# zouyuoz/SVS-UNet-PyTorch

Measured on AMD Instinct MI355X. Metric: spectrogram-tiles/sec (512x128) U-Net fwd+bwd (L1 train step incl. Adam), higher is better.
Workload: dtype f32; 1 GPU; train.py L1-loss step, 512x128 tiles, batch 64 per GPU; global_batch=64, parallelism=dp1, mode=train

## Files before the change

### svs_unet_pytorch_amd/csrc/gemm_conv.hip

```cpp
#include <stdlib.h>
#include <string.h>

#include <mutex>
#include <type_traits>
#include <vector>
#include "common.h"
#include "mfma_split.h"

enum { MODE_GATHER = 0, MODE_PARITY = 1 };

struct ConvGemmArgs {
  const float* x; long ldx;
  int B, H, W, C;
  const float* wp;
  const float* bias;
  const float* scale;
  const float* shift;
  float slope;
  float* y; long ldy;
  int Ho, Wo, N;
  int accumulate;
  int ksplit;
  float* slab;
  int tap_inner;
  int cpt_shift;
  float* stats;
};

struct ConvBal {
  int enabled;
  int npos[4];
  unsigned first[4][65];
  unsigned char nsplit[4][64];
  unsigned char* rowsplit;
};
struct ConvNoBal {};

__device__ __forceinline__ int swz(int row, int chunk) { return chunk ^ ((row >> 1) & 3); }

template <int MODE, int BM, int BN, int WM, int WN, bool SKIP = false, bool SPLIT = false, int PF = 1>
__global__ __launch_bounds__(256) void conv_gemm_kernel(ConvGemmArgs p, std::conditional_t<SKIP, ConvBal, ConvNoBal> bal) {
  constexpr int TM = BM / WM / 16;
  constexpr int TN = BN / WN / 16;
  constexpr int RA = (BM + 63) / 64;
  constexpr int RB = (BN + 63) / 64;
  static_assert(WM * WN == 4, "4 waves");
  static_assert(TM >= 1 && TN >= 1, "tile");

  __shared__ __attribute__((aligned(16))) float As[2][BM * 16];
  __shared__ __attribute__((aligned(16))) float Bs[2][BN * 16];

  const int t = threadIdx.x;
  const int lane = t & 63, wave = t >> 6;
  const int wm = wave / WN, wn = wave % WN;
  const int lrow = lane & 15, q = lane >> 4;

  int bx = blockIdx.x, by = blockIdx.y, bz = blockIdx.z;
  int nsplit = p.ksplit;
  bool balanced = false;
  if constexpr (SKIP) {
    if (bal.enabled) {
      balanced = true;
      const unsigned bid = blockIdx.x;
      int c = 0;
      if (MODE == MODE_PARITY) c = (bid >= bal.first[1][0]) + (bid >= bal.first[2][0]) + (bid >= bal.first[3][0]);
      const unsigned f = lane < bal.npos[c] ? bal.first[c][lane] : 0xFFFFFFFFu;
      const int pos = __builtin_amdgcn_readfirstlane(__builtin_popcountll(__ballot(f <= bid)) - 1);
      nsplit = bal.nsplit[c][pos];
      const int ntn = p.N / BN, per = nsplit * ntn;
      const int within = (int)(bid - bal.first[c][pos]);
      const int i = within / per, rem = within - i * per;
      by = rem / ntn;
      bx = (pos * (p.B / BM) + i) * ntn + (rem - by * ntn);
      bz = c;
    }
  }
  int ph = 0, pw = 0, nth = 5, ntw = 5;
  int Ha, Wa;
  const float* wp = p.wp;
  if (MODE == MODE_PARITY) {
    const int par = bz;
    ph = par >> 1; pw = par & 1;
    nth = 3 - ph; ntw = 3 - pw;
    Ha = (p.Ho - ph + 1) >> 1; Wa = (p.Wo - pw + 1) >> 1;
    const int poff = (par == 0) ? 0 : (par == 1) ? 9 : (par == 2) ? 15 : 21;
    wp += (long)poff * p.N * p.C;
  } else {
    Ha = p.Ho; Wa = p.Wo;
  }
  const int ntaps = nth * ntw;
  const long M = (long)p.B * Ha * Wa;
  const int ntile_n = p.N / BN;
  const long m0 = (long)(bx / ntile_n) * BM;
  const int n0 = (bx % ntile_n) * BN;
  if (m0 >= M) {
    if (p.stats && p.ksplit == 1) {
      float* out = p.stats + ((long)bz * (gridDim.x / ntile_n) + bx / ntile_n) * 2 * p.N + n0;
      for (int c = threadIdx.x; c < BN; c += 256) { out[c] = 0.f; out[p.N + c] = 0.f; }
    }
    return;
  }
  const int cpt = p.C >> 4;
  const int nkt = ntaps * cpt;
  int kt_begin = (int)((long)nkt * by / nsplit);
  int kt_end = (int)((long)nkt * (by + 1) / nsplit);
  const long Kw = (long)ntaps * p.C;

  const int chunk = t & 3;
  constexpr unsigned OOB = 0x80000000u;
  unsigned a_voff[RA], a_mask[RA];
#pragma unroll
  for (int r = 0; r < RA; ++r) {
    const int row = (t >> 2) + 64 * r;
    const long m = m0 + row;
    const bool ok = (row < BM) && (m < M);
    const long mm = ok ? m : 0;
    int wq, hq; long b;
    if (SKIP) {
      const unsigned pos = (unsigned)mm / (unsigned)p.B;
      b = (long)((unsigned)mm - pos * (unsigned)p.B);
      wq = (int)(pos / (unsigned)Ha);
      hq = (int)(pos - (unsigned)wq * (unsigned)Ha);
    } else {
      const unsigned um = (unsigned)mm, utmp = um / (unsigned)Wa;
      wq = (int)(um - utmp * (unsigned)Wa);
      const unsigned ub = utmp / (unsigned)Ha;
      hq = (int)(utmp - ub * (unsigned)Ha);
      b = ub;
    }
    const int h0 = (MODE == MODE_GATHER) ? 2 * hq : hq;
    const int w0 = (MODE == MODE_GATHER) ? 2 * wq : wq;
    a_voff[r] = ok ? (unsigned)((((b * p.H + h0) * p.W + w0) * p.ldx + chunk * 4) * 4) : OOB;
    unsigned mask = 0;
    for (int th = 0; th < nth; ++th)
      for (int tw = 0; tw < ntw; ++tw) {
        const int ih = (MODE == MODE_GATHER) ? h0 - 2 + th : h0 + 1 - th;
        const int iw = (MODE == MODE_GATHER) ? w0 - 2 + tw : w0 + 1 - tw;
        if (ok && (unsigned)ih < (unsigned)p.H && (unsigned)iw < (unsigned)p.W) mask |= 1u << (th * ntw + tw);
      }
    a_mask[r] = mask;
  }
  unsigned umask = 0x1FFFFFFu;
  if (SKIP) {
    __shared__ unsigned umask_s;
    if (t == 0) umask_s = 0;
    __syncthreads();
    unsigned mine = 0;
#pragma unroll
    for (int r = 0; r < RA; ++r) mine |= a_mask[r];
    if (mine) atomicOr(&umask_s, mine);
    __syncthreads();
    umask = __builtin_amdgcn_readfirstlane(umask_s);
    if (balanced) {
      const int nvk = __builtin_popcount(umask) << p.cpt_shift;
      const int vb = (int)((long)nvk * by / nsplit), ve = (int)((long)nvk * (by + 1) / nsplit);
      auto kt_of = [&](int v) -> int {
        unsigned m = umask;
        for (int r = v >> p.cpt_shift; r > 0; --r) m &= m - 1;
        return (__builtin_ctz(m) << p.cpt_shift) | (v & (cpt - 1));
      };
      kt_begin = vb < nvk ? kt_of(vb) : nkt;
      kt_end = ve < nvk ? kt_of(ve) : nkt;
    }
  }
  unsigned b_voff[RB];
#pragma unroll
  for (int r = 0; r < RB; ++r) {
    const int row = (t >> 2) + 64 * r;
    b_voff[r] = (row < BN) ? (unsigned)(((long)(n0 + row) * Kw + chunk * 4) * 4) : OOB;
  }
  const long shift = (MODE == MODE_GATHER) ? (2L * p.W + 2) * p.ldx : (1L * p.W + 1) * p.ldx;
  const __amdgpu_buffer_rsrc_t rx = __builtin_amdgcn_make_buffer_rsrc((void*)(p.x - shift), 0, OOB, 0x00020000);
  const __amdgpu_buffer_rsrc_t rw = __builtin_amdgcn_make_buffer_rsrc((void*)wp, 0, OOB, 0x00020000);

  f32x4 ra[RA], rb[RB];
  f32x4 ra2[PF == 2 ? RA : 1], rb2[PF == 2 ? RB : 1];
  auto load_tile_to = [&](int kt, f32x4 (&ra)[RA], f32x4 (&rb)[RB]) __attribute__((always_inline)) {
    int tap, cc;
    if (SKIP || !p.tap_inner) {
      if (p.cpt_shift >= 0) { tap = kt >> p.cpt_shift; cc = kt & (cpt - 1); }
      else { tap = kt / cpt; cc = kt - tap * cpt; }
    } else {
      cc = (ntaps == 25) ? kt / 25 : (ntaps == 9) ? kt / 9 : (ntaps == 6) ? kt / 6 : kt >> 2;
      tap = kt - cc * ntaps;
    }
    const int th = (ntw == 5) ? tap / 5 : (ntw == 3) ? tap / 3 : tap >> 1;
    const int tw = tap - th * ntw;
    const int pix = (MODE == MODE_GATHER) ? th * p.W + tw : (2 - th) * p.W + (2 - tw);
    const int soff_a = __builtin_amdgcn_readfirstlane((int)((pix * p.ldx + (cc << 4)) * 4));
    const int soff_b = __builtin_amdgcn_readfirstlane((int)(((long)tap * p.C + (cc << 4)) * 4));
#pragma unroll
    for (int r = 0; r < RA; ++r) {
      const unsigned vo = ((a_mask[r] >> tap) & 1u) ? a_voff[r] : OOB;
      ra[r] = __builtin_bit_cast(f32x4, __builtin_amdgcn_raw_buffer_load_b128(rx, (int)vo, soff_a, 0));
    }
#pragma unroll
    for (int r = 0; r < RB; ++r)
      rb[r] = __builtin_bit_cast(f32x4, __builtin_amdgcn_raw_buffer_load_b128(rw, (int)b_voff[r], soff_b, 0));
  };
  auto load_tile = [&](int kt) __attribute__((always_inline)) { load_tile_to(kt, ra, rb); };
  auto store_tile_from = [&](int buf, const f32x4 (&ra)[RA], const f32x4 (&rb)[RB]) __attribute__((always_inline)) {
#pragma unroll
    for (int r = 0; r < RA; ++r) {
      const int row = (t >> 2) + 64 * r;
      if (BM % 64 == 0 || row < BM) *(f32x4*)(&As[buf][row * 16 + swz(row, chunk) * 4]) = ra[r];
    }
#pragma unroll
    for (int r = 0; r < RB; ++r) {
      const int row = (t >> 2) + 64 * r;
      if (BN % 64 == 0 || row < BN) *(f32x4*)(&Bs[buf][row * 16 + swz(row, chunk) * 4]) = rb[r];
    }
  };

  auto store_tile = [&](int buf) __attribute__((always_inline)) { store_tile_from(buf, ra, rb); };
  f32x4 acc[TM][TN];
#pragma unroll
  for (int i = 0; i < TM; ++i)
#pragma unroll
    for (int j = 0; j < TN; ++j) acc[i][j] = (f32x4){0.f, 0.f, 0.f, 0.f};

  auto first_valid = [&](int k) -> int {
    if (!SKIP || k >= kt_end) return k;
    const int tp = k >> p.cpt_shift;
    if ((umask >> tp) & 1u) return k;
    const unsigned rest = umask >> (tp + 1);
    if (!rest) return kt_end;
    const int nk = (tp + 1 + __builtin_ctz(rest)) << p.cpt_shift;
    return nk < kt_end ? nk : kt_end;
  };
  auto multiply = [&](int buf) __attribute__((always_inline)) {
    f32x4 fa[TM], fb[TN];
#pragma unroll
    for (int i = 0; i < TM; ++i) {
      const int row = wm * (TM * 16) + i * 16 + lrow;
      fa[i] = *(const f32x4*)(&As[buf][row * 16 + swz(row, q) * 4]);
    }
#pragma unroll
    for (int j = 0; j < TN; ++j) {
      const int row = wn * (TN * 16) + j * 16 + lrow;
      fb[j] = *(const f32x4*)(&Bs[buf][row * 16 + swz(row, q) * 4]);
    }
    if constexpr (SPLIT) {
      SvsSplitA sa[TM];
      SvsSplitB sb[TN];
#pragma unroll
      for (int i = 0; i < TM; ++i) sa[i] = svs_split_a(fa[i][0], fa[i][1], fa[i][2], fa[i][3]);
// ... 34 lines not shown
    }
  } else {
  if (kt_cur < kt_end) {
    load_tile(kt_cur);
    store_tile(0);
  }
  __syncthreads();
  for (int it = 0; kt_cur < kt_end; ++it) {
    const int buf = it & 1;
    const int kt_next = first_valid(kt_cur + 1);
    const bool more = kt_next < kt_end;
    if (more) load_tile(kt_next);
    kt_cur = kt_next;
    f32x4 fa[TM], fb[TN];
#pragma unroll
    for (int i = 0; i < TM; ++i) {
      const int row = wm * (TM * 16) + i * 16 + lrow;
      fa[i] = *(const f32x4*)(&As[buf][row * 16 + swz(row, q) * 4]);
    }
#pragma unroll
    for (int j = 0; j < TN; ++j) {
      const int row = wn * (TN * 16) + j * 16 + lrow;
      fb[j] = *(const f32x4*)(&Bs[buf][row * 16 + swz(row, q) * 4]);
    }
    if constexpr (SPLIT) {
      SvsSplitA sa[TM];
      SvsSplitB sb[TN];
#pragma unroll
      for (int i = 0; i < TM; ++i) sa[i] = svs_split_a(fa[i][0], fa[i][1], fa[i][2], fa[i][3]);
#pragma unroll
      for (int j = 0; j < TN; ++j) sb[j] = svs_split_b(fb[j][0], fb[j][1], fb[j][2], fb[j][3]);
      svs_mma_split<TM, TN>(acc, sa, sb);
    } else {
#pragma unroll
      for (int k = 0; k < 4; ++k)
#pragma unroll
        for (int i = 0; i < TM; ++i)
#pragma unroll
          for (int j = 0; j < TN; ++j)
            acc[i][j] = __builtin_amdgcn_mfma_f32_16x16x4f32(fa[i][k], fb[j][k], acc[i][j], 0, 0, 0);
    }
    if (more) store_tile(buf ^ 1);
    __syncthreads();
  }
  }

  const bool split = p.ksplit > 1;
  float ssum[TN], ssq[TN];
#pragma unroll
  for (int j = 0; j < TN; ++j) { ssum[j] = 0.f; ssq[j] = 0.f; }
  float* const slab = split ? p.slab + (long)by * ((long)p.B * p.Ho * p.Wo) * p.N : nullptr;
  bool mark_rows = false;
  if constexpr (SKIP) mark_rows = balanced && by == 0 && n0 == 0 && wn == 0;
#pragma unroll
  for (int i = 0; i < TM; ++i) {
#pragma unroll
    for (int r = 0; r < 4; ++r) {
      const long m = m0 + wm * (TM * 16) + i * 16 + q * 4 + r;
      if (m >= M) continue;
      long opix;
      if (SKIP) {
        const unsigned pos = (unsigned)m / (unsigned)p.B;
        const long b = (long)((unsigned)m - pos * (unsigned)p.B);
        const int wq = (int)(pos / (unsigned)Ha);
        const int hq = (int)(pos - (unsigned)wq * (unsigned)Ha);
        opix = (MODE == MODE_GATHER) ? (b * p.Ho + hq) * p.Wo + wq : (b * p.Ho + 2 * hq + ph) * p.Wo + 2 * wq + pw;
      } else if (MODE == MODE_GATHER) {
        opix = m;
      } else {
        const unsigned um = (unsigned)m, utmp = um / (unsigned)Wa;
        const int wq = (int)(um - utmp * (unsigned)Wa);
        const unsigned ub = utmp / (unsigned)Ha;
        const int hq = (int)(utmp - ub * (unsigned)Ha);
        const long b = ub;
        opix = (b * p.Ho + 2 * hq + ph) * p.Wo + 2 * wq + pw;
      }
      if constexpr (SKIP) { if (mark_rows && lrow == 0) bal.rowsplit[opix] = (unsigned char)nsplit; }
#pragma unroll
      for (int j = 0; j < TN; ++j) {
        const int n = n0 + wn * (TN * 16) + j * 16 + lrow;
        float v = acc[i][j][r];
        if (split) {
          slab[opix * p.N + n] = v;
        } else {
          if (p.bias) v += p.bias[n];
          if (p.scale) {
            v = v * p.scale[n] + p.shift[n];
            v = v > 0.f ? v : v * p.slope;
          }
          float* dst = p.y + opix * p.ldy + n;
          if (p.accumulate) v += *dst;
          *dst = v;
          ssum[j] += v;
          ssq[j] += v * v;
        }
      }
    }
  }
  if (p.stats && !split) {
    __shared__ float st[2][WM][BN];
#pragma unroll
    for (int j = 0; j < TN; ++j) {
      ssum[j] += __shfl_xor(ssum[j], 16, 64); ssum[j] += __shfl_xor(ssum[j], 32, 64);
      ssq[j] += __shfl_xor(ssq[j], 16, 64); ssq[j] += __shfl_xor(ssq[j], 32, 64);
      if (q == 0) { st[0][wm][wn * (TN * 16) + j * 16 + lrow] = ssum[j]; st[1][wm][wn * (TN * 16) + j * 16 + lrow] = ssq[j]; }
    }
    __syncthreads();
    float* out = p.stats + ((long)bz * (gridDim.x / ntile_n) + bx / ntile_n) * 2 * p.N + n0;
    for (int c = t; c < BN; c += 256) {
      float a = 0.f, b2 = 0.f;
#pragma unroll
      for (int w = 0; w < WM; ++w) { a += st[0][w][c]; b2 += st[1][w][c]; }
      out[c] = a;
      out[p.N + c] = b2;
    }
  }
}

template <int MODE, int TM, int TN>
__global__ __launch_bounds__(256) void conv_direct_kernel(ConvGemmArgs p) {
  const int t = threadIdx.x;
  const int lane = t & 63, wave = t >> 6;
  const int lrow = lane & 15, q = lane >> 4;
  int ph = 0, pw = 0, nth = 5, ntw = 5, Ha, Wa;
  const float* wp = p.wp;
  if (MODE == MODE_PARITY) {
    const int par = blockIdx.y;
    ph = par >> 1; pw = par & 1;
    nth = 3 - ph; ntw = 3 - pw;
    Ha = (p.Ho - ph + 1) >> 1; Wa = (p.Wo - pw + 1) >> 1;
    const int poff = (par == 0) ? 0 : (par == 1) ? 9 : (par == 2) ? 15 : 21;
    wp += (long)poff * p.N * p.C;
  } else {
    Ha = p.Ho; Wa = p.Wo;
  }
  const int ntaps = nth * ntw;
  const long M = (long)p.B * Ha * Wa;
  const long m0 = ((long)blockIdx.x * 4 + wave) * (TM * 16);
  if (m0 >= M) return;
  const int cpt = p.C >> 4;
  const int nkt = ntaps * cpt;
  const long Kw = (long)ntaps * p.C;
  constexpr unsigned OOB = 0x80000000u;

  unsigned a_voff[TM], a_mask[TM];
#pragma unroll
  for (int i = 0; i < TM; ++i) {
    const long m = m0 + i * 16 + lrow;
    const bool ok = m < M;
    const long mm = ok ? m : 0;
// ... 456 lines not shown
#pragma unroll
    for (int i = 0; i < 4; ++i) acc[i] = (f32x4){0.f, 0.f, 0.f, 0.f};
    f32x4 fw[2];
    fw[0] = __builtin_bit_cast(f32x4, __builtin_amdgcn_raw_buffer_load_b128(rw, (int)w_voff, 0, 0));
    svs_static_for<25>([&](auto tc) {
      constexpr int tap = decltype(tc)::value, kh = tap / 5, kw = tap % 5;
      if constexpr (tap + 1 < 25) fw[(tap + 1) & 1] = __builtin_bit_cast(f32x4, __builtin_amdgcn_raw_buffer_load_b128(rw, (int)w_voff, (tap + 1) * 16 * 4, 0));
      f32x4 fp[4];
#pragma unroll
      for (int i = 0; i < 4; ++i) fp[i] = *(const f32x4*)(pbase + (((2 * i + kh) * 2 + (kw & 1)) * PW + (kw >> 1)) * LP);
#pragma unroll
      for (int k = 0; k < 4; ++k)
#pragma unroll
        for (int i = 0; i < 4; ++i) acc[i] = __builtin_amdgcn_mfma_f32_16x16x4f32(fw[tap & 1][k], fp[i][k], acc[i], 0, 0, 0);
    });
#pragma unroll
    for (int i = 0; i < 4; ++i) {
      const int oh = oh0 + 4 * rh + i, ow = ow0 + lrow;
      if (oh >= p.Ho || ow >= p.Wo) continue;
      f32x4 v = acc[i];
      if (p.bias) v += b4;
      if (p.scale) {
        v = v * sc4 + sh4;
#pragma unroll
        for (int k = 0; k < 4; ++k) v[k] = v[k] > 0.f ? v[k] : v[k] * p.slope;
      }
      *(f32x4*)(p.y + ((b * p.Ho + oh) * p.Wo + ow) * p.ldy + n) = v;
      s0 += v;
      s1 += v * v;
    }
  }
  if (p.stats) {
#pragma unroll
    for (int k = 0; k < 4; ++k)
#pragma unroll
      for (int o = 1; o < 16; o <<= 1) { s0[k] += __shfl_xor(s0[k], o, 64); s1[k] += __shfl_xor(s1[k], o, 64); }
    if (lrow == 0) {
#pragma unroll
      for (int k = 0; k < 4; ++k) { st[0][rh][n + k] = s0[k]; st[1][rh][n + k] = s1[k]; }
    }
    __syncthreads();
    if (t < 64) {
      const int which = t >> 5, c = t & 31;
      p.stats[(long)blockIdx.x * 64 + which * 32 + c] = st[which][0][c] + st[which][1][c];
    }
  }
}

enum ConvKind { CONV_GEMM, CONV_GATHER_WINDOW, CONV_PARITY_WINDOW, CONV_DIRECT };
struct ConvPlan {
  int kind;
  int cfg, BM, BN, WM, WN, pf;
  bool skip, split;
  long mtiles; int grid_y;
  int wC, wCW, wTN, wNT;
  bool wvec;
  int tpb, gtiles;
  dim3 grid;
  int ksplit;
  ConvBal bal;
  size_t slab_bytes, rowtab_bytes;
  long stat_rows;
};

static void plan_gemm_tile(int mode, long Mmax, int N, int nkt_min, bool narrow, bool inference, ConvPlan& pl) {
  if (N % 128 == 0) {
    if (Mmax <= 96) { pl.cfg = 4; pl.BM = 32; pl.BN = 128; }
    else { pl.cfg = 0; pl.BM = 128; pl.BN = 128; }
  } else if (N == 64) {
    if (Mmax <= 512 || nkt_min <= 25 || (inference && Mmax <= 16384)) { pl.cfg = 5; pl.BM = 64; pl.BN = 64; }
    else { pl.cfg = 1; pl.BM = 128; pl.BN = 64; }
  } else if (N == 32) { pl.cfg = 2; pl.BM = 256; pl.BN = 32; }
  else { pl.cfg = 3; pl.BM = 256; pl.BN = 16; }
  if (mode == MODE_PARITY && N % 64 == 0 && Mmax > 1024) { pl.cfg = 5; pl.BM = 64; pl.BN = 64; }
  if (narrow && N % 64 == 0) { pl.cfg = 5; pl.BM = 64; pl.BN = 64; }
  if (narrow && N == 128 && !(inference && Mmax < (mode == MODE_PARITY ? 2048 : 8192))) { pl.cfg = 6; pl.BM = 64; pl.BN = 128; }
  if (narrow && mode == MODE_GATHER && N == 256 && nkt_min == 200 && Mmax >= 4096 && Mmax % 64 == 0 && !inference) { pl.cfg = 6; pl.BM = 64; pl.BN = 128; }
  pl.split = svs_tune(SVS_TUNE_MFMA_SPLIT) > 0;
  if (pl.split && Mmax > 96) {
    if (N % 128 == 0) {
      if (mode == MODE_GATHER && Mmax >= 4096) { pl.cfg = 0; pl.BM = 128; pl.BN = 128; }
      else { pl.cfg = 6; pl.BM = 64; pl.BN = 128; }
    } else if (N == 64 && Mmax >= 16384) { pl.cfg = 1; pl.BM = 128; pl.BN = 64; }
  }
  if (svs_tune_on(SVS_TUNE_CONV_CFG)) {
    static const int bm[7] = {128, 128, 256, 256, 32, 64, 64}, bn[7] = {128, 64, 32, 16, 128, 64, 128};
    const int c = (int)svs_tune(SVS_TUNE_CONV_CFG);
    if (c >= 0 && c < 7 && N % bn[c] == 0) { pl.cfg = c; pl.BM = bm[c]; pl.BN = bn[c]; }
  }
  static const int wm[7] = {2, 2, 4, 4, 1, 2, 2};
  pl.WM = wm[pl.cfg];
  pl.WN = 4 / pl.WM;
  pl.mtiles = (Mmax + pl.BM - 1) / pl.BM;
  pl.grid_y = (mode == MODE_PARITY) ? 4 : 1;
  const long blocks = pl.mtiles * (N / pl.BN) * pl.grid_y;
  int ks = 1;
  const long target = (mode == MODE_PARITY) ? 1024 : ((inference || pl.split) ? 512 : 768);
  if (blocks < ((mode == MODE_PARITY) ? 768 : 384)) {
    ks = (int)((target + blocks - 1) / blocks);
    const int per = (mode == MODE_GATHER) ? 16 : 8;
    const int cap = nkt_min / per > 1 ? nkt_min / per : 1;
    if (ks > cap) ks = cap;
    if (ks > 64) ks = 64;
    if (ks < 1) ks = 1;
  }
  if (svs_tune_on(SVS_TUNE_CONV_KSPLIT)) { int f = (int)svs_tune(SVS_TUNE_CONV_KSPLIT); if (f >= 1 && f <= nkt_min) ks = f; }
// ... 100 lines not shown
  SVS_REQUIRE(N >= 16 && (N == 16 || N == 32 || N == 64 || N % 128 == 0), "%s: unsupported N=%d", who, N);
  SVS_REQUIRE(ldx >= C && ldx % 4 == 0 && ldy >= N, "%s: bad ld (ldx=%ld ldy=%ld)", who, ldx, ldy);
  SVS_REQUIRE(svs_aligned16(x) && svs_aligned16(wp), "%s: pointers must be 16-byte aligned", who);
  return SVS_OK;
}

static ConvPlan plan_conv_call(int mode, int B, int H, int W, int C, int Ho, int Wo, int N, long ldx, bool inference, bool accumulate,
                               bool gemm_only = false) {
  ConvPlan p{};
  const long Mmax = (mode == MODE_GATHER) ? (long)B * Ho * Wo : (long)B * ((Ho + 1) / 2) * ((Wo + 1) / 2);
  const int nkt_min = (mode == MODE_GATHER ? 25 : 4) * (C / 16);
  const long P = (long)B * Ho * Wo;
  const bool view_32bit = ((long)B * H * W * ldx + 4L * (W + 2) * ldx) * 4 < (1L << 31);
  const bool image_32bit = ((long)H * W * ldx) * 4 < (1L << 31);
  p.ksplit = 1;
  const long gtiles = (long)B * ((Ho + 7) / 8) * ((Wo + 15) / 16);
  const long gw = svs_tune(SVS_TUNE_CONV_GWINDOW);
  if (!gemm_only && mode == MODE_GATHER && C == 16 && N == 32 && !accumulate && gw != 0 && image_32bit &&
      (gw == 2  || (Ho >= 8 && Wo >= 16 && gtiles >= 256)) && gtiles < (1L << 30)) {
    const long tblocks = gw >= 16 ? gw : 512;
    int tpb = (int)(gtiles / tblocks);
    if (tpb < 1) tpb = 1;
    if (tpb > 8) tpb = 8;
    p.kind = CONV_GATHER_WINDOW;
    p.tpb = tpb; p.gtiles = (int)gtiles;
    p.grid = dim3((unsigned)((gtiles + tpb - 1) / tpb));
    p.stat_rows = p.grid.x;
    return p;
  }
  const long cw = svs_tune(SVS_TUNE_CONV_WINDOW);
  const bool pw_eligible = mode == MODE_PARITY && (N == 16 || N == 32) && (C == 32 || C == 64 || C == 128) && image_32bit;
  const long wtiles = (long)B * ((H + 7) / 8) * ((W + 15) / 16);
  const bool fills_gpu = H >= 8 && W >= 16 && wtiles >= 128;
  if (!gemm_only && pw_eligible && cw != 0 && (fills_gpu || cw == 2 || cw == 3)) {
    p.kind = CONV_PARITY_WINDOW;
    p.wC = C; p.wCW = C == 32 ? 32 : 64;
    p.grid = dim3((unsigned)wtiles);
    if (N == 32 && wtiles <= 256 && cw != 3) { p.wTN = 1; p.wNT = 2; p.grid.y = 2; }
    else { p.wTN = N / 16; p.wNT = N / 16; }
    p.stat_rows = p.grid.x;
    return p;
  }
  if (!gemm_only && Mmax >= 16384 && view_32bit && (N == 16 || (N == 32 && mode == MODE_PARITY && C >= 128))) {
    p.kind = CONV_DIRECT;
    p.grid = dim3((unsigned)((Mmax + 255) / 256), mode == MODE_PARITY ? 4 : 1);
    return p;
  }
  p.kind = CONV_GEMM;
  const long cs = svs_tune(SVS_TUNE_CONV_SKIP);
  const bool narrow_shape = N > 32 && (C & (C - 1)) == 0 && B >= 16 && ((mode == MODE_GATHER) ? Wo : (Wo + 1) / 2) <= 8;
  plan_gemm_tile(mode, Mmax, N, nkt_min, narrow_shape && cs < 0, inference, p);
  const bool can_skip = N > 32  && (C & (C - 1)) == 0 && p.BN >= 64;
  p.skip = cs == 0 ? false : cs == 2 ? can_skip : can_skip && narrow_shape;
  p.grid = dim3((unsigned)(p.mtiles * (N / p.BN)), (unsigned)p.ksplit, (unsigned)p.grid_y);
  const int slabs = p.skip ? plan_balance(mode, B, H, W, C, Ho, Wo, N, p.BM, p.BN, p.ksplit, &p.bal) : 0;
  if (slabs) {
    p.ksplit = slabs;
    p.grid = dim3(p.bal.first[p.grid_y - 1][p.bal.npos[p.grid_y - 1]], 1, 1);
    p.rowtab_bytes = svs_align_up((size_t)P, 16);
  }
  if (p.ksplit > 1) p.slab_bytes = (size_t)p.ksplit * P * N * sizeof(float);
  else p.stat_rows = p.mtiles * p.grid_y;
  return p;
}

template <int MODE, bool SPLIT, int BM, int BN, int WM, int WN>
static void launch_conv_gemm_tile(const ConvGemmArgs& a, const ConvPlan& p, hipStream_t stream) {
  constexpr int PF2 = (BM == 128 && BN == 128) || BM == 32 ? 1 : 2;
  if constexpr (BN >= 64) {
    if (p.skip) {
      if (p.pf == 2) hipLaunchKernelGGL((conv_gemm_kernel<MODE, BM, BN, WM, WN, true, SPLIT, PF2>), p.grid, dim3(256), 0, stream, a, p.bal);
      else hipLaunchKernelGGL((conv_gemm_kernel<MODE, BM, BN, WM, WN, true, SPLIT, 1>), p.grid, dim3(256), 0, stream, a, p.bal);
      return;
    }
  }
  if (p.pf == 2) hipLaunchKernelGGL((conv_gemm_kernel<MODE, BM, BN, WM, WN, false, SPLIT, PF2>), p.grid, dim3(256), 0, stream, a, ConvNoBal{});
  else hipLaunchKernelGGL((conv_gemm_kernel<MODE, BM, BN, WM, WN, false, SPLIT, 1>), p.grid, dim3(256), 0, stream, a, ConvNoBal{});
}
template <int MODE, bool SPLIT>
static void launch_conv_gemm_cfg(const ConvGemmArgs& a, const ConvPlan& p, hipStream_t stream) {
  switch (p.cfg) {
    case 0: launch_conv_gemm_tile<MODE, SPLIT, 128, 128, 2, 2>(a, p, stream); break;
    case 1: launch_conv_gemm_tile<MODE, SPLIT, 128, 64, 2, 2>(a, p, stream); break;
    case 2: launch_conv_gemm_tile<MODE, SPLIT, 256, 32, 4, 1>(a, p, stream); break;
    case 3: launch_conv_gemm_tile<MODE, SPLIT, 256, 16, 4, 1>(a, p, stream); break;
    case 4: launch_conv_gemm_tile<MODE, SPLIT, 32, 128, 1, 4>(a, p, stream); break;
    case 6: launch_conv_gemm_tile<MODE, SPLIT, 64, 128, 2, 2>(a, p, stream); break;
    default: launch_conv_gemm_tile<MODE, SPLIT, 64, 64, 2, 2>(a, p, stream); break;
  }
}
template <int MODE>
static void launch_conv_plan(const ConvGemmArgs& a, const ConvPlan& p, hipStream_t stream) {
  switch (p.kind) {
    case CONV_GATHER_WINDOW: hipLaunchKernelGGL(gather_window_kernel, p.grid, dim3(256), 0, stream, a, p.gtiles, p.tpb); break;
    case CONV_PARITY_WINDOW:
#define SVS_LAUNCH_WINDOW(C_, CW_, TN_, NT_)                                                                              \
  do {                                                                                                                   \
    if (p.wvec) hipLaunchKernelGGL((parity_window_kernel<C_, CW_, TN_, NT_, true>), p.grid, dim3(256), 0, stream, a);    \
    else hipLaunchKernelGGL((parity_window_kernel<C_, CW_, TN_, NT_, false>), p.grid, dim3(256), 0, stream, a);          \
  } while (0)
      if (p.wNT == 1) {
        if (p.wC == 32) SVS_LAUNCH_WINDOW(32, 32, 1, 1); else if (p.wC == 64) SVS_LAUNCH_WINDOW(64, 64, 1, 1); else SVS_LAUNCH_WINDOW(128, 64, 1, 1);
      } else if (p.wTN == 1) {
        if (p.wC == 32) SVS_LAUNCH_WINDOW(32, 32, 1, 2); else if (p.wC == 64) SVS_LAUNCH_WINDOW(64, 64, 1, 2); else SVS_LAUNCH_WINDOW(128, 64, 1, 2);
      } else {
        if (p.wC == 32) SVS_LAUNCH_WINDOW(32, 32, 2, 2); else if (p.wC == 64) SVS_LAUNCH_WINDOW(64, 64, 2, 2); else SVS_LAUNCH_WINDOW(128, 64, 2, 2);
      }
#undef SVS_LAUNCH_WINDOW
      break;
    case CONV_DIRECT:
      if (a.N == 16) hipLaunchKernelGGL((conv_direct_kernel<MODE, 4, 1>), p.grid, dim3(256), 0, stream, a);
      else hipLaunchKernelGGL((conv_direct_kernel<MODE, 4, 2>), p.grid, dim3(256), 0, stream, a);
      break;
    default:
      if (p.split) launch_conv_gemm_cfg<MODE, true>(a, p, stream);
      else launch_conv_gemm_cfg<MODE, false>(a, p, stream);
  }
}

int svs_conv_gemm_run(int mode, const float* x, long ldx, int B, int H, int W, int C, const float* wp,
                      const float* bias, const float* scale, const float* shift, float slope, float* y, long ldy,
                      int Ho, int Wo, int N, int accumulate, void* ws, size_t ws_bytes, hipStream_t stream,
                      const char* who, float* stats, int stats_cap, int* stats_nblk) {
  if (stats_nblk) *stats_nblk = 0;
  int rc = check_gemm_args(who, x, ldx, B, H, W, C, wp, y, ldy, Ho, Wo, N);
  if (rc) return rc;
  if (mode == MODE_GATHER)
    SVS_REQUIRE(Ho == svs_conv_out(H) && Wo == svs_conv_out(W), "%s: output %dx%d does not match input %dx%d", who, Ho, Wo, H, W);
  else
    SVS_REQUIRE((Ho == 2 * H || Ho == 2 * H - 1) && (Wo == 2 * W || Wo == 2 * W - 1),
// ... 22 lines not shown
  const bool want_stats = stats && stats_nblk && !scale && !accumulate;
  if (want_stats && p.stat_rows && p.stat_rows * 2 * N <= stats_cap) { a.stats = stats; *stats_nblk = (int)p.stat_rows; }
  if (mode == MODE_GATHER) launch_conv_plan<MODE_GATHER>(a, p, stream);
  else launch_conv_plan<MODE_PARITY>(a, p, stream);
  static const char* const kernel[4] = {"conv_gemm", "gather_window", "parity_window", "conv_direct"};
  SVS_CHECK_LAUNCH(kernel[p.kind]);
  if (p.ksplit == 1 || svs_tune_flag(SVS_TUNE_SKIP_REDUCE)) return SVS_OK;
  const long P = (long)B * Ho * Wo, total4 = P * N / 4;
  int grid = (int)((total4 + 255) / 256);
  if (grid > 2048) grid = 2048;
  const bool fuse = stats && stats_nblk && stats_cap >= 2 * N && N % 4 == 0 && N <= 1024 && 256 % (N / 4) == 0 && !scale && !accumulate;
  if (fuse && grid > 512) grid = 512;
  if (fuse && (long)grid * 2 * N > stats_cap) grid = stats_cap / (2 * N);
  int n_shift = -1;
  if ((N & (N - 1)) == 0) { n_shift = 0; while ((1 << n_shift) < N) ++n_shift; }
  if (fuse && N % 32 == 0 && svs_tune(SVS_TUNE_BN_INLINE) != 0) {
    const int nslab = N / 32;
    long rows = 512 / nslab;
    if (rows > (P + 31) / 32) rows = (P + 31) / 32;
    if (rows * 2 * N > stats_cap) rows = stats_cap / (2 * N);
    if (rows < 1) rows = 1;
    const long ppr = (P + rows - 1) / rows;
    rows = (P + ppr - 1) / ppr;
    hipLaunchKernelGGL(splitk_epilogue_stats_kernel, dim3((unsigned)(rows * nslab)), dim3(256), 0, stream, a.slab, p.ksplit, P, N, bias,
                       y, ldy, stats, ppr, p.bal.enabled ? p.bal.rowsplit : nullptr);
    SVS_CHECK_LAUNCH("splitk_epilogue_stats");
    *stats_nblk = (int)rows;
    return SVS_OK;
  }
  hipLaunchKernelGGL(splitk_epilogue_kernel, dim3(grid), dim3(256), 0, stream, a.slab, p.ksplit, P, N, bias, scale,
                     shift, slope, y, ldy, accumulate, fuse ? stats : nullptr, n_shift, p.bal.enabled ? p.bal.rowsplit : nullptr);
  SVS_CHECK_LAUNCH("splitk_epilogue");
  if (fuse) *stats_nblk = grid;
  return SVS_OK;
}

size_t svs_conv_gemm_workspace(int mode, int B, int H, int W, int C, int Ho, int Wo, int N) {
  if (C < 16 || N < 16) return 0;
  size_t need = 0;
  for (int inference = 0; inference < 2; ++inference) {
    const ConvPlan p = plan_conv_call(mode, B, H, W, C, Ho, Wo, N, C, inference != 0, false, true);
    need = p.slab_bytes + p.rowtab_bytes > need ? p.slab_bytes + p.rowtab_bytes : need;
  }
  return need;
}

int svs_conv_gemm_describe(int mode, int B, int H, int W, int C, int Ho, int Wo, int N, long ldx, char* buf, size_t n) {
  const ConvPlan p = plan_conv_call(mode, B, H, W, C, Ho, Wo, N, ldx, false, false);
  switch (p.kind) {
    case CONV_GATHER_WINDOW: snprintf(buf, n, "gather_window_kernel"); break;
    case CONV_PARITY_WINDOW: snprintf(buf, n, "parity_window_kernel<%d, %d, %d, %d, true>", p.wC, p.wCW, p.wTN, p.wNT); break;
    case CONV_DIRECT: snprintf(buf, n, "conv_direct_kernel<%d, 4, %d>", mode, N / 16); break;
    default:
      snprintf(buf, n, "conv_gemm_kernel<%d, %d, %d, %d, %d, %s, %s, %d>", mode, p.BM, p.BN, p.WM, p.WN, p.skip ? "true" : "false",
               p.split ? "true" : "false", p.pf);
  }
  return p.ksplit;
}
```

### svs_unet_pytorch_amd/csrc/net.hip

```cpp
#include <math.h>
#include <algorithm>
#include <atomic>
#include <mutex>
#include <stdarg.h>
#include <stdlib.h>
#include <string.h>

#include "unet_desc.h"

static thread_local char g_err[512] = "";
void svs_set_error(const char* fmt, ...) {
  va_list ap;
  va_start(ap, fmt);
  vsnprintf(g_err, sizeof(g_err), fmt, ap);
  va_end(ap);
}
extern "C" const char* svs_last_error_string(void) { return g_err; }

static const char* const TUNE_NAMES[SVS_TUNE_COUNT] = {
    "CONV_CFG", "CONV_KSPLIT", "CONV_WINDOW", "CONV_SKIP", "SKIP_REDUCE", "WGRAD_CFG", "WGRAD_KSPLIT", "WGRAD_SKIP",
    "WGRAD_WINDOW", "TRAIN_UNFUSED", "TRAIN_ONE_STREAM", "MFMA_SPLIT", "CONV_C1_TILED", "BF16_CFG", "BF16_KSPLIT", "BN_INLINE",
    "CONV_GWINDOW"};
static std::atomic<long> g_tune[SVS_TUNE_COUNT];
static std::once_flag g_tune_once;
// ... 235 lines not shown
  float* dbias_part[11];
  float* scratch; size_t scratch_bytes;
  float* scratch2; size_t scratch2_bytes;
  size_t total;
};
#define SVS_FUSED_STATS_ROWS 512
static TrainWs train_layout(const Geo& g, void* ws) {
  TrainWs t{};
  Arena a{(char*)ws, 0};
  auto take = [&](size_t nfloats) { return a.take<float>(nfloats); };
  for (int k = 1; k <= 5; ++k) t.cat[k] = take((size_t)g.P[k] * 2 * CH[k]);
  t.c6 = take((size_t)g.P[6] * CH[6]);
  for (int l = 0; l < 11; ++l) t.raw[l] = take((size_t)g.P[bn_level(l)] * bn_channels(l));
  for (int l = 0; l < 11; ++l) { t.mean[l] = take(bn_channels(l)); t.invstd[l] = take(bn_channels(l)); }
  for (int l = 1; l <= 10; ++l) { t.wfwd[l] = take(param_numel(4 * l)); t.wbwd[l] = take(param_numel(4 * l)); }
  for (int k = 1; k <= 5; ++k) t.dcat[k] = take((size_t)g.P[k] * 2 * CH[k]);
  t.dc6 = take((size_t)g.P[6] * CH[6]);
  size_t dmax = 0;
  for (int k = 1; k <= 6; ++k) if ((size_t)g.P[k] * CH[k] > dmax) dmax = (size_t)g.P[k] * CH[k];
  t.d_raw = take(dmax);
  for (int l = 0; l < 11; ++l) t.d_raw_l[l] = take((size_t)g.P[bn_level(l)] * bn_channels(l));
  t.d_logit = take((size_t)g.P[0]);
  t.mask = take((size_t)g.P[0]);
  size_t bb = 0;
  for (int k = 1; k <= 6; ++k) { size_t s = svs_bn_workspace_bytes(g.P[k], CH[k]); if (s > bb) bb = s; }
  if (bb < (size_t)SVS_FUSED_STATS_ROWS * 2 * CH[6] * sizeof(float)) bb = (size_t)SVS_FUSED_STATS_ROWS * 2 * CH[6] * sizeof(float);
  t.bnws_bytes = bb + 4096;
  t.bnws = take(t.bnws_bytes / sizeof(float));
  for (int l = 0; l < 11; ++l) t.dbias_part[l] = take(svs_bn_partial_floats(g.P[bn_level(l)], bn_channels(l)));
  t.scratch2_bytes = max_layer_bytes(0, 11, [&](const Layer& L) { return bwd_weight_ws(g, L); });
  t.scratch_bytes = std::max({(size_t)4096, t.scratch2_bytes,
                              max_layer_bytes(1, 10, [&](const Layer& L) { return std::max(fwd_ws(g, L), bwd_data_ws(g, L)); })});
  t.scratch = take(t.scratch_bytes / sizeof(float) + 64);
  t.scratch2 = take(t.scratch2_bytes / sizeof(float) + 64);
  t.total = a.used;
  return t;
}

struct SideStream { hipStream_t s; hipEvent_t fork[4], done[4], sync; int nfork; std::mutex mu; };
static SideStream* g_side[64] = {};
static std::mutex g_side_mutex;
static SideStream* side_stream(hipStream_t of) {
  int dev = 0;
  hipDevice_t sdev;
  if (of && hipStreamGetDevice(of, &sdev) == hipSuccess) dev = (int)sdev;
  else if (hipGetDevice(&dev) != hipSuccess) return nullptr;
  if (dev < 0 || dev >= 64) return nullptr;
  std::lock_guard<std::mutex> lock(g_side_mutex);
  if (!g_side[dev]) {
    SideStream* sd = new SideStream();
    int least = 0, greatest = 0;
    bool ok = hipDeviceGetStreamPriorityRange(&least, &greatest) == hipSuccess;
    ok = ok && hipStreamCreateWithPriority(&sd->s, hipStreamNonBlocking, greatest) == hipSuccess;
    ok = ok && hipEventCreateWithFlags(&sd->sync, hipEventDisableTiming) == hipSuccess;
    for (int i = 0; i < 4 && ok; ++i)
      ok = hipEventCreateWithFlags(&sd->fork[i], hipEventDisableTiming) == hipSuccess &&
           hipEventCreateWithFlags(&sd->done[i], hipEventDisableTiming) == hipSuccess;
    if (!ok) { delete sd; return nullptr; }
    g_side[dev] = sd;
  }
  return g_side[dev];
}

extern "C" size_t svs_unet_train_workspace_bytes(int B, int H, int W) {
  Geo g;
  if (make_geo(B, H, W, g)) return 0;
  return train_layout(g, nullptr).total;
}

struct WsName { const char* stem; int first, count; float* const* p; };
static int64_t ws_find(const WsName* tab, size_t n, const char* name, const char* base) {
  for (size_t i = 0; i < n; ++i) {
    const size_t len = strlen(tab[i].stem);
    if (strncmp(name, tab[i].stem, len)) continue;
    if (!tab[i].count) {
      if (!name[len]) return (const char*)*tab[i].p - base;
      continue;
    }
    char* end;
    const long idx = strtol(name + len, &end, 10) - tab[i].first;
    if (end != name + len && !*end && idx >= 0 && idx < tab[i].count) return (const char*)tab[i].p[idx] - base;
  }
  return -1;
}
extern "C" int64_t svs_unet_ws_offset(const char* name, int B, int H, int W, int training) {
  Geo g;
  if (!name || make_geo(B, H, W, g)) return -1;
  if (training == 2) return svs_unet_bf16_ws_offset(name, g);
  char* const base = (char*)256;
  if (training) {
    const TrainWs t = train_layout(g, base);
    const WsName tab[] = {{"cat", 1, 5, t.cat + 1}, {"c6", 0, 0, &t.c6},         {"raw_e", 1, 6, t.raw},  {"raw_d", 1, 5, t.raw + 6},
                          {"dcat", 1, 5, t.dcat + 1}, {"dc6", 0, 0, &t.dc6},     {"d_logit", 0, 0, &t.d_logit}, {"mask", 0, 0, &t.mask},
                          {"mean", 0, 11, t.mean},  {"invstd", 0, 11, t.invstd}};
    return ws_find(tab, sizeof(tab) / sizeof(tab[0]), name, base);
  }
  const EvalWs e = eval_layout(g, base);
  const WsName tab[] = {{"cat", 1, 5, e.cat + 1}, {"c6", 0, 0, &e.c6}};
  return ws_find(tab, sizeof(tab) / sizeof(tab[0]), name, base);
}

struct TrainCall { Geo g; TrainWs t; ParamView v; };
static int train_prologue(const char* who, const float* params, int B, int H, int W, void* ws, size_t ws_bytes, TrainCall& c) {
  const int rc = make_geo(B, H, W, c.g);
  if (rc) return rc;
  c.t = train_layout(c.g, ws);
  if (!ws || ws_bytes < c.t.total || !svs_aligned16(ws)) {
    svs_set_error("%s: workspace too small (%zu < %zu)", who, ws_bytes, c.t.total);
    return SVS_ERR_WORKSPACE;
  }
// ... 276 lines not shown
```

Measured before the change: 19500 tiles/s.

## Add position-uniform tap-skip conv GEMM variant and lighter side-stream events

Adds a UNI template form of the tap-skipping conv GEMM. It is used when every row of an M tile shares one spatial position, which holds when B is a multiple of BM. In that form the tap mask is computed once per tile instead of per row, which drops the shared-memory atomicOr reduction and its two barriers, the per-row masks in the load path, and the generic epilogue indexing, replacing it with a strided per-image store. Separately, the side-stream fork and join events are created with hipEventDisableSystemFence to cut synchronisation overhead. The risks are extra template instantiations and correctness depending on the batch-major row ordering assumption.

```diff
diff --git a/svs_unet_pytorch_amd/csrc/gemm_conv.hip b/svs_unet_pytorch_amd/csrc/gemm_conv.hip
--- a/svs_unet_pytorch_amd/csrc/gemm_conv.hip
+++ b/svs_unet_pytorch_amd/csrc/gemm_conv.hip
@@ -38,8 +38,9 @@
 
 __device__ __forceinline__ int swz(int row, int chunk) { return chunk ^ ((row >> 1) & 3); }
 
-template <int MODE, int BM, int BN, int WM, int WN, bool SKIP = false, bool SPLIT = false, int PF = 1>
+template <int MODE, int BM, int BN, int WM, int WN, bool UNI, bool SKIP, bool SPLIT, int PF>
 __global__ __launch_bounds__(256) void conv_gemm_kernel(ConvGemmArgs p, std::conditional_t<SKIP, ConvBal, ConvNoBal> bal) {
+  static_assert(SKIP || !UNI, "the position-uniform form is a form of the tap-skipping kernel");
   constexpr int TM = BM / WM / 16;
   constexpr int TN = BN / WN / 16;
   constexpr int RA = (BM + 63) / 64;
@@ -58,6 +59,7 @@
   int bx = blockIdx.x, by = blockIdx.y, bz = blockIdx.z;
   int nsplit = p.ksplit;
   bool balanced = false;
+  int upos = -1, ub0 = 0;
   if constexpr (SKIP) {
     if (bal.enabled) {
       balanced = true;
@@ -73,6 +75,7 @@
       by = rem / ntn;
       bx = (pos * (p.B / BM) + i) * ntn + (rem - by * ntn);
       bz = c;
+      upos = pos; ub0 = i * BM;
     }
   }
   int ph = 0, pw = 0, nth = 5, ntw = 5;
@@ -109,6 +112,35 @@
   const int chunk = t & 3;
   constexpr unsigned OOB = 0x80000000u;
   unsigned a_voff[RA], a_mask[RA];
+  unsigned umask = 0x1FFFFFFu;
+  int uhq = 0, uwq = 0;
+  if constexpr (UNI) {
+    if (upos < 0) {
+      upos = (int)((unsigned)m0 / (unsigned)p.B);
+      ub0 = (int)((unsigned)m0 - (unsigned)upos * (unsigned)p.B);
+    }
+    uwq = (int)((unsigned)upos / (unsigned)Ha);
+    uhq = upos - uwq * Ha;
+    const int h0 = (MODE == MODE_GATHER) ? 2 * uhq : uhq, w0 = (MODE == MODE_GATHER) ? 2 * uwq : uwq;
+    unsigned wbits = 0;
+    for (int tw = 0; tw < ntw; ++tw) {
+      const int iw = (MODE == MODE_GATHER) ? w0 - 2 + tw : w0 + 1 - tw;
+      if ((unsigned)iw < (unsigned)p.W) wbits |= 1u << tw;
+    }
+    umask = 0;
+    for (int th = 0; th < nth; ++th) {
+      const int ih = (MODE == MODE_GATHER) ? h0 - 2 + th : h0 + 1 - th;
+      if ((unsigned)ih < (unsigned)p.H) umask |= wbits << (th * ntw);
+    }
+    const unsigned base = (unsigned)((((long)h0 * p.W + w0) * p.ldx + chunk * 4) * 4);
+    const unsigned per_image = (unsigned)(((long)p.H * p.W * p.ldx) * 4);
+#pragma unroll
+    for (int r = 0; r < RA; ++r) {
+      const int row = (t >> 2) + 64 * r;
+      a_voff[r] = (BM % 64 == 0 || row < BM) ? base + (unsigned)(ub0 + row) * per_image : OOB;
+      a_mask[r] = 0;
+    }
+  } else {
 #pragma unroll
   for (int r = 0; r < RA; ++r) {
     const int row = (t >> 2) + 64 * r;
@@ -140,17 +172,19 @@
       }
     a_mask[r] = mask;
   }
-  unsigned umask = 0x1FFFFFFu;
+  }
   if (SKIP) {
-    __shared__ unsigned umask_s;
-    if (t == 0) umask_s = 0;
-    __syncthreads();
-    unsigned mine = 0;
-#pragma unroll
-    for (int r = 0; r < RA; ++r) mine |= a_mask[r];
-    if (mine) atomicOr(&umask_s, mine);
-    __syncthreads();
-    umask = __builtin_amdgcn_readfirstlane(umask_s);
+    if constexpr (!UNI) {
+      __shared__ unsigned umask_s;
+      if (t == 0) umask_s = 0;
+      __syncthreads();
+      unsigned mine = 0;
+#pragma unroll
+      for (int r = 0; r < RA; ++r) mine |= a_mask[r];
+      if (mine) atomicOr(&umask_s, mine);
+      __syncthreads();
+      umask = __builtin_amdgcn_readfirstlane(umask_s);
+    }
     if (balanced) {
       const int nvk = __builtin_popcount(umask) << p.cpt_shift;
       const int vb = (int)((long)nvk * by / nsplit), ve = (int)((long)nvk * (by + 1) / nsplit);
@@ -191,7 +225,7 @@
     const int soff_b = __builtin_amdgcn_readfirstlane((int)(((long)tap * p.C + (cc << 4)) * 4));
 #pragma unroll
     for (int r = 0; r < RA; ++r) {
-      const unsigned vo = ((a_mask[r] >> tap) & 1u) ? a_voff[r] : OOB;
+      const unsigned vo = (UNI || ((a_mask[r] >> tap) & 1u)) ? a_voff[r] : OOB;
       ra[r] = __builtin_bit_cast(f32x4, __builtin_amdgcn_raw_buffer_load_b128(rx, (int)vo, soff_a, 0));
     }
 #pragma unroll
@@ -332,6 +366,47 @@
   float* const slab = split ? p.slab + (long)by * ((long)p.B * p.Ho * p.Wo) * p.N : nullptr;
   bool mark_rows = false;
   if constexpr (SKIP) mark_rows = balanced && by == 0 && n0 == 0 && wn == 0;
+  if constexpr (UNI) {
+    const long HoWo = (long)p.Ho * p.Wo;
+    const long pix0 = ((MODE == MODE_GATHER) ? (long)uhq * p.Wo + uwq : (long)(2 * uhq + ph) * p.Wo + 2 * uwq + pw) +
+                      (long)(ub0 + wm * (TM * 16) + q * 4) * HoWo;
+    const int ncol = n0 + wn * (TN * 16) + lrow;
+    const long rstride = HoWo * (split ? (long)p.N : p.ldy);
+    float* const out = split ? slab + pix0 * p.N + ncol : p.y + pix0 * p.ldy + ncol;
+    float cb[TN], csc[TN], csh[TN];
+#pragma unroll
+    for (int j = 0; j < TN; ++j) {
+      cb[j] = (!split && p.bias) ? p.bias[ncol + j * 16] : 0.f;
+      csc[j] = (!split && p.scale) ? p.scale[ncol + j * 16] : 0.f;
+      csh[j] = (!split && p.scale) ? p.shift[ncol + j * 16] : 0.f;
+    }
+#pragma unroll
+    for (int i = 0; i < TM; ++i) {
+#pragma unroll
+      for (int r = 0; r < 4; ++r) {
+        if (mark_rows && lrow == 0) bal.rowsplit[pix0 + (i * 16 + r) * HoWo] = (unsigned char)nsplit;
+        float* const row = out + (i * 16 + r) * rstride;
+#pragma unroll
+        for (int j = 0; j < TN; ++j) {
+          float v = acc[i][j][r];
+          if (split) {
+            row[j * 16] = v;
+          } else {
+            if (p.bias) v += cb[j];
+            if (p.scale) {
+              v = v * csc[j] + csh[j];
+              v = v > 0.f ? v : v * p.slope;
+            }
+            float* dst = row + j * 16;
+            if (p.accumulate) v += *dst;
+            *dst = v;
+            ssum[j] += v;
+            ssq[j] += v * v;
+          }
+        }
+      }
+    }
+  } else {
 #pragma unroll
   for (int i = 0; i < TM; ++i) {
 #pragma unroll
@@ -376,6 +451,7 @@
         }
       }
     }
+  }
   }
   if (p.stats && !split) {
     __shared__ float st[2][WM][BN];
@@ -938,6 +1014,7 @@
   int kind;
   int cfg, BM, BN, WM, WN, pf;
   bool skip, split;
+  bool uni;
   long mtiles; int grid_y;
   int wC, wCW, wTN, wNT;
   bool wvec;
@@ -1144,6 +1221,7 @@
   plan_gemm_tile(mode, Mmax, N, nkt_min, narrow_shape && cs < 0, inference, p);
   const bool can_skip = N > 32  && (C & (C - 1)) == 0 && p.BN >= 64;
   p.skip = cs == 0 ? false : cs == 2 ? can_skip : can_skip && narrow_shape;
+  p.uni = p.skip && B % p.BM == 0 && !p.split && p.cfg != 0;
   p.grid = dim3((unsigned)(p.mtiles * (N / p.BN)), (unsigned)p.ksplit, (unsigned)p.grid_y);
   const int slabs = p.skip ? plan_balance(mode, B, H, W, C, Ho, Wo, N, p.BM, p.BN, p.ksplit, &p.bal) : 0;
   if (slabs) {
@@ -1160,14 +1238,20 @@
 static void launch_conv_gemm_tile(const ConvGemmArgs& a, const ConvPlan& p, hipStream_t stream) {
   constexpr int PF2 = (BM == 128 && BN == 128) || BM == 32 ? 1 : 2;
   if constexpr (BN >= 64) {
+    if constexpr (!SPLIT && !(BM == 128 && BN == 128)) {
+      if (p.uni) {
+        hipLaunchKernelGGL((conv_gemm_kernel<MODE, BM, BN, WM, WN, true, true, false, PF2>), p.grid, dim3(256), 0, stream, a, p.bal);
+        return;
+      }
+    }
     if (p.skip) {
-      if (p.pf == 2) hipLaunchKernelGGL((conv_gemm_kernel<MODE, BM, BN, WM, WN, true, SPLIT, PF2>), p.grid, dim3(256), 0, stream, a, p.bal);
-      else hipLaunchKernelGGL((conv_gemm_kernel<MODE, BM, BN, WM, WN, true, SPLIT, 1>), p.grid, dim3(256), 0, stream, a, p.bal);
+      if (p.pf == 2) hipLaunchKernelGGL((conv_gemm_kernel<MODE, BM, BN, WM, WN, false, true, SPLIT, PF2>), p.grid, dim3(256), 0, stream, a, p.bal);
+      else hipLaunchKernelGGL((conv_gemm_kernel<MODE, BM, BN, WM, WN, false, true, SPLIT, 1>), p.grid, dim3(256), 0, stream, a, p.bal);
       return;
     }
   }
-  if (p.pf == 2) hipLaunchKernelGGL((conv_gemm_kernel<MODE, BM, BN, WM, WN, false, SPLIT, PF2>), p.grid, dim3(256), 0, stream, a, ConvNoBal{});
-  else hipLaunchKernelGGL((conv_gemm_kernel<MODE, BM, BN, WM, WN, false, SPLIT, 1>), p.grid, dim3(256), 0, stream, a, ConvNoBal{});
+  if (p.pf == 2) hipLaunchKernelGGL((conv_gemm_kernel<MODE, BM, BN, WM, WN, false, false, SPLIT, PF2>), p.grid, dim3(256), 0, stream, a, ConvNoBal{});
+  else hipLaunchKernelGGL((conv_gemm_kernel<MODE, BM, BN, WM, WN, false, false, SPLIT, 1>), p.grid, dim3(256), 0, stream, a, ConvNoBal{});
 }
 template <int MODE, bool SPLIT>
 static void launch_conv_gemm_cfg(const ConvGemmArgs& a, const ConvPlan& p, hipStream_t stream) {
@@ -1296,8 +1380,8 @@
     case CONV_PARITY_WINDOW: snprintf(buf, n, "parity_window_kernel<%d, %d, %d, %d, true>", p.wC, p.wCW, p.wTN, p.wNT); break;
     case CONV_DIRECT: snprintf(buf, n, "conv_direct_kernel<%d, 4, %d>", mode, N / 16); break;
     default:
-      snprintf(buf, n, "conv_gemm_kernel<%d, %d, %d, %d, %d, %s, %s, %d>", mode, p.BM, p.BN, p.WM, p.WN, p.skip ? "true" : "false",
-               p.split ? "true" : "false", p.pf);
+      snprintf(buf, n, "conv_gemm_kernel<%d, %d, %d, %d, %d, %s, %s, %s, %d>", mode, p.BM, p.BN, p.WM, p.WN, p.uni ? "true" : "false",
+               p.skip ? "true" : "false", p.split ? "true" : "false", p.pf);
   }
   return p.ksplit;
 }
diff --git a/svs_unet_pytorch_amd/csrc/net.hip b/svs_unet_pytorch_amd/csrc/net.hip
--- a/svs_unet_pytorch_amd/csrc/net.hip
+++ b/svs_unet_pytorch_amd/csrc/net.hip
@@ -311,10 +311,11 @@
     int least = 0, greatest = 0;
     bool ok = hipDeviceGetStreamPriorityRange(&least, &greatest) == hipSuccess;
     ok = ok && hipStreamCreateWithPriority(&sd->s, hipStreamNonBlocking, greatest) == hipSuccess;
-    ok = ok && hipEventCreateWithFlags(&sd->sync, hipEventDisableTiming) == hipSuccess;
+    const unsigned flags = hipEventDisableTiming | hipEventDisableSystemFence;
+    ok = ok && hipEventCreateWithFlags(&sd->sync, flags) == hipSuccess;
     for (int i = 0; i < 4 && ok; ++i)
-      ok = hipEventCreateWithFlags(&sd->fork[i], hipEventDisableTiming) == hipSuccess &&
-           hipEventCreateWithFlags(&sd->done[i], hipEventDisableTiming) == hipSuccess;
+      ok = hipEventCreateWithFlags(&sd->fork[i], flags) == hipSuccess &&
+           hipEventCreateWithFlags(&sd->done[i], flags) == hipSuccess;
     if (!ok) { delete sd; return nullptr; }
     g_side[dev] = sd;
   }
```

New measurement: 20190 tiles/s, median of 6. 3.5% higher.
